# learningmatter-mit/surface-sampling

Measured on AMD Instinct MI355X. Metric: MC energy-evaluations/sec (SrTiO3(001) ~250-atom slabs, 3-model PaiNN ensemble E+F incl. neighbor list), higher is better.
Workload: dtype f32 via fp16x2-split MFMA (3 products), fp32 accumulate; neighbor decisions f64; 1 GPU; SrTiO3(001) PaiNN x3, 256 batched independent chains per GPU (BASELINE configs[3]), 248-272 atoms/chain; chains_per_gpu=256, atoms_per_gpu=66503, edges_per_gpu=2747786, slots_per_gpu=2836316, models=3, streams_per_gpu=2, parallelism=one GPU, no collective

## Files before the change

surface-sampling_amd/csrc/painn.hip:

```cpp
#include "vssr_internal.h"

namespace vssr {

constexpr int T = NODE_TILE;
constexpr int RB = 21;
constexpr int ECHUNK = 16;
constexpr float PI_F = 3.14159265358979323846f;

__device__ inline float sigmoidf_(float x) { return 1.f / (1.f + expf(-x)); }
__device__ inline float swishf_(float x) { return x * sigmoidf_(x); }
__device__ inline float dswishf_(float x) {
    float sg = sigmoidf_(x);
    return sg * fmaf(x, 1.f - sg, 1.f);
}

__global__ void __launch_bounds__(128) k_embed(int N, const int *__restrict__ Z, const ModelW *__restrict__ MW,
                                               float *__restrict__ s0, float *__restrict__ v0) {
    int i = blockIdx.x, m = blockIdx.y, f = threadIdx.x;
    const ModelW &W = MW[m];
    size_t a = (size_t)m * N + i;
    s0[a * F + f] = W.embed[(size_t)Z[i] * F + f];
    v0[(a * 3 + 0) * F + f] = 0.f;
    v0[(a * 3 + 1) * F + f] = 0.f;
    v0[(a * 3 + 2) * F + f] = 0.f;
// ... 509 lines not shown
    return painn_alloc_results(h);
}

int painn_alloc_results(vssr_handle *h) {
    const size_t N = h->n_atoms, M = h->n_models;
    if (h->d_energy.ensure(sizeof(float) * h->n_cfg) || h->d_energy_std.ensure(sizeof(float) * h->n_cfg) ||
        h->d_energy_models.ensure(sizeof(float) * h->n_cfg * M) || h->d_energy64.ensure(sizeof(double) * h->n_cfg * (2 + M)) ||
        h->d_forces.ensure(sizeof(float) * 3 * N) ||
        h->d_forces_std.ensure(sizeof(float) * 3 * N) || h->d_e_atoms.ensure(sizeof(float) * N))
        return set_err(h, VSSR_E_NOMEM, "result buffers: out of device memory");
    if (h->d_sat.bytes < sizeof(unsigned) * h->n_cfg || h->d_sat_out.bytes < sizeof(unsigned) * h->n_cfg) {
        if (h->d_sat.ensure(sizeof(unsigned) * h->n_cfg) || h->d_sat_out.ensure(sizeof(unsigned) * h->n_cfg))
            return set_err(h, VSSR_E_NOMEM, "saturation flags: out of device memory");
        VSSR_HIP(h, hipMemsetAsync(h->d_sat.p, 0, h->d_sat.bytes, h->stream));
        VSSR_HIP(h, hipMemsetAsync(h->d_sat_out.p, 0, h->d_sat_out.bytes, h->stream));
    }
    return VSSR_OK;
}

int painn_run(vssr_handle *h, uint32_t want) {
    if (h->painn_general) return painn_gen_run(h, want);
    const int N = h->n_atoms, M = h->n_models, L = h->num_conv, H = h->readout_hidden;
    hipStream_t st = h->stream;
    h->h_sat_valid = false;
    int rc = build_neighbors(h, (double)h->cutoff);
    if (rc) return rc;
    rc = painn_alloc_state(h);
    if (rc) return rc;
    StateView &sv = h->sv;
    sv.e_excl = h->d_excl.as<float>();
    const GraphView G = graph_view(h);
    const ActiveView &av = G.act;
    const ModelW *MW = h->model_table.as<ModelW>();
    const int *counters = h->d_counters.as<int>();
    const int *Z = h->d_Z.as<int>();
    dim3 blk(128);
    dim3 g_atom(N, M), g_tile((N + T - 1) / T, M);
    Profiler &P = h->prof;
    const bool l0_fact = h->l0_enabled && h->l0_nz > 0;
    const int n_groups = painn_gbar_groups(h);
    const bool partial = n_groups > 1;
    const int layer_sets = partial ? L - 1 : 1, per_set = n_groups / layer_sets;
    const int *cls_list[EDGE_MFMA_CLASSES];
    const int *bcls_list[EDGE_MFMA_BCLASSES];
    {
        int o = 0;
        for (int c = 0; c < EDGE_MFMA_CLASSES; o += h->n_class[c], ++c) cls_list[c] = h->d_class_list.as<int>() + o;
        for (int c = 0; c < EDGE_MFMA_BCLASSES; o += h->n_bclass[c], ++c) bcls_list[c] = h->d_class_list.as<int>() + o;
    }
    const int n_gather = h->n_class[EDGE_CLASS_GATHER];
    const bool keep = h->upd_save && (want & VSSR_WANT_FORCES) && readout_mfma_supported(H);
    auto save_of = [&](int l) -> void * { return keep ? (char *)h->d_upd_save.p + update_save_bytes(N, M) * (size_t)l : nullptr; };
    h->l0_used = l0_fact;

    if (!l0_fact) {
        P.begin(KC_EMBED, st);
        hipLaunchKernelGGL(k_embed, g_atom, blk, 0, st, N, Z, MW, sv.s_in[0], sv.v_in[0]);
        P.end(st);
    }
    for (int l = 0; l < L; ++l) {
        if (l == 0 && l0_fact) {
            P.begin(KC_L0_FWD, st);
            rc = l0_run_forward(h, G, sv.s_msg[0], sv.v_msg[0]);
            if (rc) return rc;
            P.end(st);
            P.begin(KC_UPDATE_FWD, st);
            launch_update_fwd_mfma(st, N, M, l, av, MW, sv.s_msg[l], sv.v_msg[l], sv.s_in[l + 1],
                                   (l + 1 < L || h->debug_keep) ? sv.v_in[l + 1] : nullptr, l + 1 < L ? sv.phi[l + 1] : nullptr, save_of(l));
            P.end(st);
            continue;
        }
        if (l == 0) {
            P.begin(KC_MSG_MLP, st);
            launch_msg_mlp_mfma(st, N, M, l, av, MW, sv.s_in[l], sv.phi[l]);
            P.end(st);
        }
        P.begin(KC_EDGE_FWD, st);
        if (l == 0)
            hipLaunchKernelGGL(k_edge_fwd<true>, g_atom, blk, 0, st, N, l, MW, G, counters, h->cutoff, h->excl_vol,
                               h->excl_sigma, h->excl_power, sv.s_in[l], sv.v_in[l], sv.phi[l], sv.s_msg[l],
                               sv.v_msg[l], -1);
        else {
            for (int cls = 0; cls < EDGE_MFMA_CLASSES; ++cls)
                launch_edge_fwd_mfma(st, cls, N, cls_list[cls], h->n_class[cls], M, l, h->max_class_atoms[cls], MW, G, counters,
                                     (int)(h->slot_cap - 1), sv.s_in[l], sv.v_in[l], sv.phi[l], sv.s_msg[l], sv.v_msg[l],
                                     (cls == EDGE_CLASS_FS4 && h->fwd_two_pass) ? h->d_bundle_sub.as<int4>() : (const int4 *)nullptr,
                                     h->fwd_two_pass, h->sub_chunk_fwd ? h->sub_chunk_fwd : sub_chunk_max(h->fwd_two_pass));
            if (n_gather)
                hipLaunchKernelGGL(k_edge_fwd<false>, g_atom, blk, 0, st, N, l, MW, G, counters, h->cutoff, h->excl_vol,
                                   h->excl_sigma, h->excl_power, sv.s_in[l], sv.v_in[l], sv.phi[l], sv.s_msg[l],
                                   sv.v_msg[l], (int)EDGE_BCLASS_GATHER);
        }
        P.end(st);
        P.begin(KC_UPDATE_FWD, st);
        launch_update_fwd_mfma(st, N, M, l, av, MW, sv.s_msg[l], sv.v_msg[l], sv.s_in[l + 1],
                               (l + 1 < L || h->debug_keep) ? sv.v_in[l + 1] : nullptr, l + 1 < L ? sv.phi[l + 1] : nullptr, save_of(l));
        P.end(st);
    }
    const bool fused = readout_mfma_supported(H);
    const bool want_forces = (want & VSSR_WANT_FORCES) != 0;
    const float *e_excl = h->excl_vol ? sv.e_excl : (const float *)nullptr;
    if (!(fused && want_forces)) {
        P.begin(KC_READOUT, st);
        if (fused) launch_readout_mfma(st, N, M, av, MW, sv.s_in[L], e_excl, sv.e_atom);
        else
            hipLaunchKernelGGL(k_readout, g_tile, blk, 0, st, N, H, av, MW, sv.s_in[L], sv.e_excl, h->excl_vol, sv.e_atom,
                               sv.sbar);
        P.end(st);
    }

    if (want_forces) {
        float *sb_buf[2] = {sv.sbar_msg, sv.sbar};
        for (int l = L - 1; l >= 0; --l) {
            float *sbar_msg_l = fused ? sb_buf[(L - 1 - l) & 1] : sv.sbar_msg;
            const float *sbar_msg_up = sb_buf[(L - l) & 1];
            P.begin(KC_UPDATE_BWD, st);
            if (!fused)
                launch_update_bwd_mfma(st, N, M, l, 0, (int)(l == L - 1), av, MW, sv.s_msg[l], sv.v_msg[l], sv.sbar, sv.vbar,
                                       nullptr, nullptr, nullptr, nullptr, sbar_msg_l, sv.vbar_msg, nullptr);
            else if (l == L - 1)
                launch_update_bwd_mfma(st, N, M, l, 1, 1, av, MW, sv.s_msg[l], sv.v_msg[l], nullptr, sv.vbar, sv.s_in[L], nullptr,
                                       e_excl, sv.e_atom, sbar_msg_l, sv.vbar_msg, save_of(l));
            else
                launch_update_bwd_mfma(st, N, M, l, 2, 0, av, MW, sv.s_msg[l], sv.v_msg[l], sbar_msg_up, sv.vbar, sv.s_in[l + 1],
                                       sv.phibar, nullptr, nullptr, sbar_msg_l, sv.vbar_msg, save_of(l));
            P.end(st);
            sv.sbar_msg_l0 = sbar_msg_l;
            P.begin((l == 0 && l0_fact) ? KC_L0_BWD : KC_EDGE_BWD, st);
            int accumulate = (l != L - 1);
            if (l == 0 && l0_fact) {
                rc = l0_run_reverse(h, G, (int)(L == 1), (int)partial, sbar_msg_l, sv.vbar_msg, sv.gbar);
                if (rc) return rc;
            } else if (l == 0)
                hipLaunchKernelGGL(k_edge_bwd<true>, g_atom, blk, 0, st, N, l, accumulate, MW, G, counters,
                                   h->cutoff, h->excl_vol, h->excl_sigma, h->excl_power, sv.v_in[l], sv.phi[l],
                                   sbar_msg_l, sv.vbar_msg, sv.phibar, sv.vbar, sv.gbar,
                                   (long long)h->slot_cap, -1, (int)partial);
            else {
                for (int cls = 0; cls < EDGE_MFMA_BCLASSES; ++cls)
                    launch_edge_bwd_mfma(st, cls, N, bcls_list[cls], h->n_bclass[cls], M, l, h->max_bclass_atoms[cls], MW, G, counters,
                                         (int)(h->slot_cap - 1), sv.v_in[l], sv.phi[l], sbar_msg_l, sv.vbar_msg, sv.phibar, sv.vbar,
                                         h->d_gpart.as<float>(), (long long)h->slot_cap, n_groups, (L - 1 - l) * per_set,
                                         cls == EDGE_BCLASS_FS16P ? h->d_bundle_subb.as<int4>() : (const int4 *)nullptr,
                                         h->sub_chunk_bwd ? h->sub_chunk_bwd : sub_chunk_max_bwd());
                if (n_gather)
                    hipLaunchKernelGGL(k_edge_bwd<false>, g_atom, blk, 0, st, N, l, accumulate, MW, G, counters,
                                       h->cutoff, h->excl_vol, h->excl_sigma, h->excl_power, sv.v_in[l], sv.phi[l],
                                       sbar_msg_l, sv.vbar_msg, sv.phibar, sv.vbar, sv.gbar,
                                       (long long)h->slot_cap, (int)EDGE_BCLASS_GATHER, 0);
            }
            P.end(st);
            if (l > 0 && !fused) {
                P.begin(KC_MSG_MLP_BWD, st);
                launch_msg_mlp_bwd_mfma(st, N, M, l, av, MW, sv.s_in[l], sv.phibar, sv.sbar_msg, sv.sbar);
                P.end(st);
            }
        }
    }
    P.begin(KC_FINALIZE, st);
    if (want_forces && partial) {
        const int uni = h->active_mask ? 0 : h->n_bclass[EDGE_BCLASS_FS16] + h->n_bclass[EDGE_BCLASS_FS16P] == h->n_cfg ? 8 : h->n_bclass[EDGE_BCLASS_FS8] == h->n_cfg ? 16
                        : h->n_bclass[EDGE_BCLASS_FS4] == h->n_cfg ? 32 : 0;
        const dim3 grid = uni ? dim3((unsigned)((h->slot_cap + 255) / 256), 1) : dim3(h->n_cfg, 12);
        hipLaunchKernelGGL(k_reduce_gpart, grid, dim3(256), 0, st, M, n_groups, layer_sets, G, counters, h->d_gpart.as<float>(),
                           sv.gbar, (long long)h->slot_cap, uni);
    }
    painn_finalize(h, G, want);
    P.end(st);
    VSSR_HIP(h, hipGetLastError());
    return VSSR_OK;
}

void painn_finalize(vssr_handle *h, const GraphView &G, uint32_t want) {
    const int N = h->n_atoms, M = h->n_models;
    hipStream_t st = h->stream;
    if (want & VSSR_WANT_FORCES)
        hipLaunchKernelGGL(k_finalize_forces, dim3((N + 3) / 4), dim3(256), 0, st, N, M, G, h->d_counters.as<int>(), h->sv.gbar,
                           (long long)h->slot_cap, h->units_per_ev, h->d_forces.as<float>(), h->d_forces_std.as<float>());
// ... 17 lines not shown
```

surface-sampling_amd/csrc/painn_node_mfma.hip:

```cpp
#include "mfma16.h"

#ifdef PHASE_TIMING
__device__ unsigned long long g_phase[64];
#define PH_INIT unsigned long long ph_t = wall_clock64();
#define PH_RESET ph_t = wall_clock64();
#define PH(k) { const unsigned long long ph_n = wall_clock64(); if (threadIdx.x == 0) atomicAdd(&g_phase[k], ph_n - ph_t); ph_t = wall_clock64(); }
extern "C" int vssr_debug_phases(unsigned long long *out, int reset) {
    if (hipMemcpyFromSymbol(out, HIP_SYMBOL(g_phase), sizeof(unsigned long long) * 64) != hipSuccess) return -1;
    if (reset) { unsigned long long z[64] = {}; if (hipMemcpyToSymbol(HIP_SYMBOL(g_phase), z, sizeof(z)) != hipSuccess) return -1; }
    return 0;
}
#else
#define PH_INIT
#define PH_RESET
#define PH(k)
#endif

namespace vssr {

template <int NRT, int NCT>
struct GemmShape {
    static constexpr int NT = NRT * NCT, NACC = NT >= 3 ? 1 : 2;
};
template <int NRT, int NCT, int NPRE>
// ... 228 lines not shown
    zero_acc(a1);
    const f32x4 b1v = gload4f(W.b1 + L.col0);
    __builtin_amdgcn_sched_barrier(0);
    {
        const uint4 *wp[1] = {WTILE(W1, L.w, F)};
        gemm16<F, 2, 1>(xs, wp, h1);
        const uint4 *wq[1] = {WTILE(W2t, L.w, F3)};
        gemm16<F3, 2, 1>(pb, wq, a1);
    }
    __syncthreads();
    {
        const f32x4 b = b1v;
#pragma unroll
        for (int t = 0; t < 2; ++t) {
            f32x4 hv;
#pragma unroll
            for (int i = 0; i < 4; ++i) hv[i] = a1[t][0][i] * dswish(h1[t][0][i] + b[i]);
            store_split4(xs, L.row(t), L.col0, hv, sat);
        }
    }
    __syncthreads();
    f32x4 acc[2][1];
    zero_acc(acc);
    const uint4 *wp[1] = {WTILE(W1t, L.w, F)};
    gemm16<F, 2, 1>(xs, wp, acc);
#pragma unroll
    for (int t = 0; t < 2; ++t) {
        const int a = a0 + L.row(t);
        if (a < N)
            *reinterpret_cast<f32x4 *>(sbar_in + (mN + a) * F + L.col0) = gload4f(sbar_msg + (mN + a) * F + L.col0) + acc[t][0];
    }
    sat.commit(av, a0, N);
}

template <int RT>
struct UpdLds {
    static constexpr int TA = 16 * RT;
    static constexpr int OFF_VT = 0;
    static constexpr int OFF_HS = plane_halves(3 * TA, F);
    static constexpr int OFF_AS = OFF_HS + plane_halves(TA, 2 * F);
    static constexpr int HALVES = OFF_AS + plane_halves(TA, F);
    static_assert(plane_halves(TA, F3) <= OFF_HS, "qb overlays vt");
    static_assert(plane_halves(3 * TA, 2 * F) <= HALVES, "[Ubar | Vbar] overlays the whole region");
};

template <int RT>
struct UpdRegs {
    f32x4 uv[3 * RT][2];
    f32x4 h3[RT];
    f32x4 gate[RT][2];
    f32x4 nrm[RT], inner[RT];
};

template <int RT, int PHB, int PF, class Sat>
__device__ __forceinline__ void update_forward(const LayerW &W, _Float16 *ldsh, const LaneGeo &L, UpdRegs<RT> &R, Sat &sat) {
    constexpr int TA = 16 * RT, OFF_VT = UpdLds<RT>::OFF_VT, OFF_HS = UpdLds<RT>::OFF_HS, OFF_AS = UpdLds<RT>::OFF_AS;
    const Planes vt = make_planes(ldsh + OFF_VT, 3 * TA, F), hs = make_planes(ldsh + OFF_HS, TA, 2 * F),
                 as_ = make_planes(ldsh + OFF_AS, TA, F);
    zero_acc(R.uv);
    PH_INIT
    {
        const uint4 *wp[2] = {WTILE(U, L.w, F), WTILE(V, L.w, F)};
        gemm16<F, 3 * RT, 2, PF>(vt, wp, R.uv);
    }
    PH(PHB + 1)
#pragma unroll
    for (int t = 0; t < RT; ++t) {
#pragma unroll
        for (int i = 0; i < 4; ++i) {
            float n2 = 0.f, in = 0.f;
#pragma unroll
            for (int x = 0; x < 3; ++x) {
                const float vv = R.uv[RT * x + t][1][i];
                n2 += fmaf(vv, vv, 1e-15f);
                in = fmaf(R.uv[RT * x + t][0][i], vv, in);
            }
            R.nrm[t][i] = sqrtf(n2);
            R.inner[t][i] = in;
        }
        store_split4(hs, L.row(t), F + L.col0, R.nrm[t], sat);
    }
    PH(PHB + 2)
    __syncthreads();
    PH(PHB + 3)
    {
        f32x4 acc[RT][1];
        zero_acc(acc);
        const uint4 *wp[1] = {WTILE(W3, L.w, 2 * F)};
        const f32x4 b = gload4f(W.b3 + L.col0);
        __builtin_amdgcn_sched_barrier(0);
        gemm16<2 * F, RT, 1, PF>(hs, wp, acc);
#pragma unroll
        for (int t = 0; t < RT; ++t) {
            R.h3[t] = acc[t][0] + b;
            f32x4 sw;
#pragma unroll
            for (int i = 0; i < 4; ++i) sw[i] = swish(R.h3[t][i]);
            store_split4(as_, L.row(t), L.col0, sw, sat);
        }
    }
    PH(PHB + 4)
    __syncthreads();
    PH(PHB + 5)
    {
        zero_acc(R.gate);
        const uint4 *wp[2] = {WTILE(W4, L.w, F), WTILE(W4, NW + L.w, F)};
        f32x4 b4[2];
#pragma unroll
        for (int c = 0; c < 2; ++c) b4[c] = gload4f(W.b4 + c * F + L.col0);
        __builtin_amdgcn_sched_barrier(0);
        gemm16<F, RT, 2, PF>(as_, wp, R.gate);
#pragma unroll
        for (int c = 0; c < 2; ++c) {
            const f32x4 b = b4[c];
#pragma unroll
            for (int t = 0; t < RT; ++t) R.gate[t][c] += b;
        }
    }
    PH(PHB + 6)
}

template <int RT, class Sat>
__device__ __forceinline__ void load_update_v(_Float16 *ldsh, const float *__restrict__ v_msg, size_t mN, int a0, int N, Sat &sat) {
    constexpr int TA = 16 * RT;
    const Planes vt = make_planes(ldsh + UpdLds<RT>::OFF_VT, 3 * TA, F);
    load_rows_split<3 * TA>(vt, 0, [&](int row) {
        int x = row / TA, a = min(a0 + (row % TA), N - 1);
        return v_msg + ((mN + a) * 3 + x) * F;
    }, sat);
}
template <int RT, class Sat>
__device__ __forceinline__ void load_update_s(_Float16 *ldsh, const float *__restrict__ s_msg, size_t mN, int a0, int N, Sat &sat) {
    constexpr int TA = 16 * RT;
    const Planes hs = make_planes(ldsh + UpdLds<RT>::OFF_HS, TA, 2 * F);
    load_rows_split<TA>(hs, 0, [&](int row) { return s_msg + (mN + min(a0 + row, N - 1)) * F; }, sat);
}

constexpr int CF_XS = plane_halves(3 * TA, F);
constexpr int CF_LDS_HALVES = CF_XS + plane_halves(TA, F);
static_assert(2 * plane_halves(TA, F) <= CF_XS, "|Vv| and swish planes overlay the v tile");
static_assert(4 * TA * FT * sizeof(float) <= CF_LDS_HALVES * sizeof(_Float16), "output tile overlays the planes");
#ifndef UPD_SAVE_LATE
#define UPD_SAVE_LATE 1
#endif
constexpr int UPD_SAVE_UV = 0, UPD_SAVE_H3 = 12, UPD_SAVE_GATE = 14, UPD_SAVE_REGS = 18;
__device__ __forceinline__ f32x4 &save_slot(f32x4 *save, int m, int k) {
    return save[(((size_t)m * gridDim.x + blockIdx.x) * UPD_SAVE_REGS + k) * NTHREADS + threadIdx.x];
}
size_t update_save_bytes(int N, int M) { return sizeof(f32x4) * (size_t)M * ((N + TA - 1) / TA) * UPD_SAVE_REGS * NTHREADS; }

template <int TAIL>
__global__ void __launch_bounds__(NTHREADS) __attribute__((amdgpu_waves_per_eu(2, 2)))
k_update_fwd_mfma(int N, int l, ActiveView av, const ModelW *__restrict__ MW, const float *__restrict__ s_msg,
                  const float *__restrict__ v_msg, float *__restrict__ s_out, float *__restrict__ v_out,
                  float *__restrict__ phi_next, f32x4 *__restrict__ save) {
    extern __shared__ __attribute__((aligned(16))) _Float16 ldsh[];
    constexpr bool NOV = TAIL == 2;
// ... 234 lines not shown
                es = fmaf(w6[i], swish(hval[i]), es);
                hb[i] = w6[i] * dswish(hval[i]);
            }
            if (WANT_SBAR) store_split4(hp, L.row(t), L.col0, hb, sat);
            es = xrow_sum_f32(es);
            if (lane < 16) red[L.w * TA + L.row(t)] = es;
        }
    }
    __syncthreads();
    if (threadIdx.x < TA) {
        const int atom = a0 + threadIdx.x;
        if (atom < N) {
            float e = gload1f(W.b6);
#pragma unroll
            for (int k = 0; k < NCW; ++k) e += red[k * TA + threadIdx.x];
            if (e_excl) e += e_excl[atom];
            e_atom[mN + atom] = e;
        }
    }
    if (WANT_SBAR) {
        f32x4 acc[RT][1];
        zero_acc(acc);
        const uint4 *wp[1] = {W.qW5t + (size_t)L.w * 4 * RH};
        gemm16<RH, RT, 1>(hp, wp, acc);
#pragma unroll
        for (int t = 0; t < RT; ++t) sb[t] = acc[t][0];
    }
}

__global__ void __launch_bounds__(NTHREADS)
k_readout_mfma(int N, ActiveView av, const ModelW *__restrict__ MW, const float *__restrict__ s, const float *__restrict__ e_excl,
               float *__restrict__ e_atom) {
    extern __shared__ __attribute__((aligned(16))) _Float16 ldsh[];
    const int m = blockIdx.y, a0 = blockIdx.x * TA;
    if (!av.tile(min(a0, N - 1), min(a0 + TA - 1, N - 1))) return;
    const LaneGeo L;
    SatTrack sat;
    const size_t mN = (size_t)m * N;
    const Planes xs = make_planes(ldsh, TA, F), hp = make_planes(ldsh + plane_halves(TA, F), TA, RH);
    float *red = reinterpret_cast<float *>(ldsh + plane_halves(TA, F) + plane_halves(TA, RH));
    load_rows_split<TA>(xs, 0, [&](int row) { return s + (mN + min(a0 + row, N - 1)) * F; }, sat);
    __syncthreads();
    f32x4 sb[2];
    readout_head<2, false>(MW[m], xs, hp, red, L, a0, N, mN, e_excl, e_atom, sb, sat);
    sat.commit(av, a0, N);
}

template <int MODE, int RT, bool SAVED = false>
__global__ void __launch_bounds__(NTHREADS) __attribute__((amdgpu_waves_per_eu(RT == 1 ? 4 : 2, RT == 1 ? 4 : 2)))
k_update_bwd_mfma(int N, int l, int vbar_is_zero, ActiveView av, const ModelW *__restrict__ MW, const float *__restrict__ s_msg,
                  const float *__restrict__ v_msg, const float *__restrict__ sbar_src, const float *__restrict__ vbar,
                  const float *__restrict__ s_next, const float *__restrict__ phibar, const float *__restrict__ e_excl,
                  float *__restrict__ e_atom, float *__restrict__ sbar_msg, float *__restrict__ vbar_msg,
                  const f32x4 *__restrict__ save) {
    static_assert(!SAVED || RT == 2, "the saved layout is that of the 32-atom forward kernel");
    extern __shared__ __attribute__((aligned(16))) _Float16 ldsh[];
    constexpr int TA = 16 * RT, OFF_VT = UpdLds<RT>::OFF_VT, OFF_AS = UpdLds<RT>::OFF_AS, UPD_LDS_HALVES = UpdLds<RT>::HALVES;
    const int m = blockIdx.y, a0 = blockIdx.x * TA;
    if (!av.tile(min(a0, N - 1), min(a0 + TA - 1, N - 1))) return;
    const LaneGeo L;
    constexpr int BPF = MODE == 0 ? 0 : UPD_PF;
    SatNone unwatched;
    const LayerW &W = MW[m].layer[l];
    const size_t mN = (size_t)m * N;
    PH_INIT
    f32x4 sb[RT];
    if (MODE != 1) {
#pragma unroll
        for (int t = 0; t < RT; ++t) sb[t] = gload4f(sbar_src + (mN + min(a0 + L.row(t), N - 1)) * F + L.col0);
    }
    float *VB = reinterpret_cast<float *>(ldsh + UPD_LDS_HALVES);
    if (MODE == 1) vbar_is_zero = 1;
    if (!vbar_is_zero) {
        constexpr int NIT = 3 * TA * (F / 4) / NTHREADS;
        float4 vv[NIT];
#pragma unroll
        for (int it = 0; it < NIT; ++it) {
            const int idx = threadIdx.x + it * NTHREADS, row = idx >> 5, c4 = idx & 31;
            vv[it] = *reinterpret_cast<const float4 *>(vbar + ((mN + min(a0 + row % TA, N - 1)) * 3 + row / TA) * F + 4 * c4);
        }
#pragma unroll
        for (int it = 0; it < NIT; ++it) {
            const int idx = threadIdx.x + it * NTHREADS, row = idx >> 5, c4 = idx & 31;
            *reinterpret_cast<float4 *>(VB + row * FT + 4 * c4) = vv[it];
        }
    }
    UpdRegs<RT> R;
    auto load_saved = [&]() {
        const f32x4 *sv = save + (((size_t)m * gridDim.x + blockIdx.x) * UPD_SAVE_REGS) * NTHREADS + threadIdx.x;
#pragma unroll
        for (int j = 0; j < 3 * RT; ++j)
#pragma unroll
            for (int c = 0; c < 2; ++c) R.uv[j][c] = gload4f(reinterpret_cast<const float *>(sv + (size_t)(UPD_SAVE_UV + 2 * j + c) * NTHREADS));
#pragma unroll
        for (int t = 0; t < RT; ++t) {
            R.h3[t] = gload4f(reinterpret_cast<const float *>(sv + (size_t)(UPD_SAVE_H3 + t) * NTHREADS));
#pragma unroll
            for (int c = 0; c < 2; ++c) R.gate[t][c] = gload4f(reinterpret_cast<const float *>(sv + (size_t)(UPD_SAVE_GATE + 2 * t + c) * NTHREADS));
        }
    };
    if (!SAVED) load_update_s<RT>(ldsh, s_msg, mN, a0, N, unwatched);
    else load_saved();
    if (MODE == 0) {
        load_update_v<RT>(ldsh, v_msg, mN, a0, N, unwatched);
        __syncthreads();
    } else if (MODE == 1) {
        if (!SAVED) load_update_v<RT>(ldsh, v_msg, mN, a0, N, unwatched);
        const Planes xs = make_planes(ldsh + OFF_AS, TA, F);
        const Planes hp = make_planes(ldsh + UPD_LDS_HALVES, TA, RH);
        float *red = reinterpret_cast<float *>(ldsh + UPD_LDS_HALVES + plane_halves(TA, RH));
        {
            SatTrack satc;
            load_rows_split<TA>(xs, 0, [&](int row) { return s_next + (mN + min(a0 + row, N - 1)) * F; }, satc);
            satc.commit(av, a0, N);
        }
        __syncthreads();
        PH(40)
        {
            SatTrack sate;
            readout_head<RT, true>(MW[m], xs, hp, red, L, a0, N, mN, e_excl, e_atom, sb, sate);
            sate.commit(av, a0, N);
        }
        PH(41)
    } else {
        const LayerW &Wn = MW[m].layer[l + 1];
        const Planes xs = make_planes(ldsh + OFF_AS, TA, F), pb = make_planes(ldsh + OFF_VT, TA, F3);
        load_rows_split<TA>(xs, 0, [&](int row) { return s_next + (mN + min(a0 + row, N - 1)) * F; }, unwatched);
        {
            SatTrack satc;
#pragma unroll
            for (int c = 0; c < 3; ++c)
                load_rows_split<TA>(pb, c * F, [&](int row) { return phibar + (mN + min(a0 + row, N - 1)) * F3 + c * F; }, satc);
            satc.commit(av, a0, N);
        }
        __syncthreads();
        PH(42)
        f32x4 h1[RT][1], a1[RT][1];
        zero_acc(h1);
        zero_acc(a1);
        const f32x4 b1n = gload4f(Wn.b1 + L.col0);
        __builtin_amdgcn_sched_barrier(0);
        {
            const uint4 *wp[1] = {Wn.qW1 + (size_t)L.w * 4 * F};
            gemm16<F, RT, 1, BPF>(xs, wp, h1);
            const uint4 *wq[1] = {Wn.qW2t + (size_t)L.w * 4 * F3};
            gemm16<F3, RT, 1, BPF>(pb, wq, a1);
        }
        PH(43)
        __syncthreads();
        if (!SAVED) load_update_v<RT>(ldsh, v_msg, mN, a0, N, unwatched);
        PH(44)
        {
            const f32x4 b = b1n;
            SatTrack sate;
#pragma unroll
            for (int t = 0; t < RT; ++t) {
                f32x4 hv;
#pragma unroll
                for (int i = 0; i < 4; ++i) hv[i] = a1[t][0][i] * dswish(h1[t][0][i] + b[i]);
                store_split4(xs, L.row(t), L.col0, hv, sate);
            }
            sate.commit(av, a0, N);
        }
        __syncthreads();
        f32x4 acc[RT][1];
        zero_acc(acc);
        const uint4 *wp[1] = {Wn.qW1t + (size_t)L.w * 4 * F};
        gemm16<F, RT, 1, BPF>(xs, wp, acc);
#pragma unroll
        for (int t = 0; t < RT; ++t) sb[t] += acc[t][0];
        PH(45)
    }
    PH(16)
    if constexpr (!SAVED) {
        update_forward<RT, 16, BPF>(W, ldsh, L, R, unwatched);
    } else {
#pragma unroll
        for (int t = 0; t < RT; ++t)
#pragma unroll
            for (int i = 0; i < 4; ++i) {
                float in = 0.f;
#pragma unroll
                for (int x = 0; x < 3; ++x) in = fmaf(R.uv[RT * x + t][0][i], R.uv[RT * x + t][1][i], in);
                R.inner[t][i] = in;
            }
        __syncthreads();
    }
    PH_RESET
    const Planes qb = make_planes(ldsh + OFF_VT, TA, F3);
    SatTrack sat;
#pragma unroll
    for (int t = 0; t < RT; ++t) {
        const int row = L.row(t);
        f32x4 abar_vv = {0.f, 0.f, 0.f, 0.f};
        if (!vbar_is_zero) {
#pragma unroll
            for (int x = 0; x < 3; ++x) {
                const f32x4 vb = *reinterpret_cast<const f32x4 *>(VB + (x * TA + row) * FT + L.col0);
#pragma unroll
                for (int i = 0; i < 4; ++i) abar_vv[i] = fmaf(vb[i], R.uv[RT * x + t][0][i], abar_vv[i]);
            }
        }
        store_split4(qb, row, L.col0, abar_vv, sat);
        store_split4(qb, row, F + L.col0, sb[t] * R.inner[t], sat);
        store_split4(qb, row, 2 * F + L.col0, sb[t], sat);
    }
    sat.commit(av, a0, N);
    sat = SatTrack();
    PH(23)
    __syncthreads();
    PH(24)
    const Planes hb = make_planes(ldsh + OFF_AS, TA, F);
    {
        f32x4 acc[RT][1];
        zero_acc(acc);
        const uint4 *wp[1] = {WTILE(W4t, L.w, F3)};
        gemm16<F3, RT, 1, BPF>(qb, wp, acc);
#pragma unroll
        for (int t = 0; t < RT; ++t) {
            f32x4 hv;
#pragma unroll
            for (int i = 0; i < 4; ++i) hv[i] = acc[t][0][i] * dswish(R.h3[t][i]);
            store_split4(hb, L.row(t), L.col0, hv, sat);
        }
        sat.commit(av, a0, N);
        sat = SatTrack();
    }
    PH(25)
// ... 79 lines not shown
void pack_mfma_tiles16(const float *Wsrc, int rows, int K, unsigned *dst) {
    auto split2 = [](float x, unsigned (&p)[2]) {
        const _Float16 h = (_Float16)x;
        const _Float16 l = (_Float16)(x - (float)h);
        unsigned short hb, lb;
        memcpy(&hb, &h, 2);
        memcpy(&lb, &l, 2);
        p[0] = hb; p[1] = lb;
    };
    const int ntile = rows / 16, nq = K / 32;
    for (int tile = 0; tile < ntile; ++tile)
        for (int q = 0; q < nq; ++q)
            for (int lane = 0; lane < 64; ++lane)
                for (int j = 0; j < 4; ++j) {
                    const size_t row = (size_t)tile * 16 + (lane & 15);
                    const int k = 32 * q + 8 * (lane >> 4) + 2 * j;
                    unsigned p0[2], p1[2];
                    split2(Wsrc[row * K + k], p0);
                    split2(Wsrc[row * K + k + 1], p1);
                    for (int pc = 0; pc < 2; ++pc)
                        dst[((((size_t)tile * nq + q) * 2 + pc) * 64 + lane) * 4 + j] = p0[pc] | (p1[pc] << 16);
                }
}

size_t node_mfma_lds_bytes(int which) {
    switch (which) {
        case 0: return sizeof(_Float16) * 2 * plane_halves(TA, F);
        case 1: return sizeof(_Float16) * (plane_halves(TA, F) + plane_halves(TA, F3));
        case 4: return sizeof(_Float16) * (plane_halves(TA, F) + plane_halves(TA, RH)) + sizeof(float) * (RH / 16) * TA;
        case 6: return 96 * 1024;
        default: return sizeof(_Float16) * UpdLds<2>::HALVES + sizeof(float) * 3 * TA * FT;
    }
}
static_assert(sizeof(_Float16) * plane_halves(16, RH) + sizeof(float) * (RH / 16) * 16 <= sizeof(float) * 3 * 16 * FT,
              "readout scratch fits the vbar region");

static_assert(sizeof(_Float16) * (CF_LDS_HALVES + plane_halves(TA, F)) <= 96 * 1024, "update fwd LDS request");

bool readout_mfma_supported(int hidden) { return hidden == RH; }

int node_mfma_init(vssr_handle *h) {
    VSSR_HIP(h, hipFuncSetAttribute((const void *)k_msg_mlp_mfma<2, 0>, hipFuncAttributeMaxDynamicSharedMemorySize, 96 * 1024));
    VSSR_HIP(h, hipFuncSetAttribute((const void *)k_msg_mlp_bwd_mfma, hipFuncAttributeMaxDynamicSharedMemorySize,
                                    (int)node_mfma_lds_bytes(1)));
    VSSR_HIP(h, hipFuncSetAttribute((const void *)k_update_fwd_mfma<0>, hipFuncAttributeMaxDynamicSharedMemorySize,
                                    (int)node_mfma_lds_bytes(6)));
    VSSR_HIP(h, hipFuncSetAttribute((const void *)k_update_fwd_mfma<1>, hipFuncAttributeMaxDynamicSharedMemorySize,
                                    (int)node_mfma_lds_bytes(6)));
    VSSR_HIP(h, hipFuncSetAttribute((const void *)k_update_fwd_mfma<2>, hipFuncAttributeMaxDynamicSharedMemorySize,
                                    (int)node_mfma_lds_bytes(6)));
#define SET_UPD(MODE)                                                                                                     \
    VSSR_HIP(h, hipFuncSetAttribute((const void *)k_update_bwd_mfma<MODE, 2>, hipFuncAttributeMaxDynamicSharedMemorySize, \
                                    (int)node_mfma_lds_bytes(3)));
    SET_UPD(0) SET_UPD(1) SET_UPD(2)
#undef SET_UPD
    VSSR_HIP(h, hipFuncSetAttribute((const void *)k_update_bwd_mfma<1, 2, true>, hipFuncAttributeMaxDynamicSharedMemorySize,
                                    (int)node_mfma_lds_bytes(3)));
    VSSR_HIP(h, hipFuncSetAttribute((const void *)k_update_bwd_mfma<2, 2, true>, hipFuncAttributeMaxDynamicSharedMemorySize,
                                    (int)node_mfma_lds_bytes(3)));
    VSSR_HIP(h, hipFuncSetAttribute((const void *)k_readout_mfma, hipFuncAttributeMaxDynamicSharedMemorySize,
                                    (int)node_mfma_lds_bytes(4)));
    return VSSR_OK;
}

void launch_msg_mlp_mfma(hipStream_t st, int N, int M, int l, const ActiveView &av, const ModelW *MW, const float *s_in,
                         float *phi) {
    hipLaunchKernelGGL((k_msg_mlp_mfma<2, 0>), dim3((N + TA - 1) / TA, M), dim3(NTHREADS), node_mfma_lds_bytes(0), st, N, l, av, MW,
                       s_in, phi);
}
void launch_msg_mlp_bwd_mfma(hipStream_t st, int N, int M, int l, const ActiveView &av, const ModelW *MW, const float *s_in,
                             const float *phibar, const float *sbar_msg, float *sbar_in) {
    hipLaunchKernelGGL(k_msg_mlp_bwd_mfma, dim3((N + TA - 1) / TA, M), dim3(NTHREADS), node_mfma_lds_bytes(1), st, N, l, av, MW,
                       s_in, phibar, sbar_msg, sbar_in);
}
void launch_update_fwd_mfma(hipStream_t st, int N, int M, int l, const ActiveView &av, const ModelW *MW, const float *s_msg,
                            const float *v_msg, float *s_out, float *v_out, float *phi_next, void *save) {
    f32x4 *sv = reinterpret_cast<f32x4 *>(save);
    if (phi_next)
        hipLaunchKernelGGL(k_update_fwd_mfma<1>, dim3((N + TA - 1) / TA, M), dim3(NTHREADS), node_mfma_lds_bytes(6), st, N, l,
                           av, MW, s_msg, v_msg, s_out, v_out, phi_next, sv);
    else if (!v_out && !sv)
        hipLaunchKernelGGL(k_update_fwd_mfma<2>, dim3((N + TA - 1) / TA, M), dim3(NTHREADS), node_mfma_lds_bytes(6), st, N, l,
                           av, MW, s_msg, v_msg, s_out, v_out, phi_next, sv);
    else
        hipLaunchKernelGGL(k_update_fwd_mfma<0>, dim3((N + TA - 1) / TA, M), dim3(NTHREADS), node_mfma_lds_bytes(6), st, N, l,
                           av, MW, s_msg, v_msg, s_out, v_out, phi_next, sv);
}
void launch_readout_mfma(hipStream_t st, int N, int M, const ActiveView &av, const ModelW *MW, const float *s,
                         const float *e_excl, float *e_atom) {
    hipLaunchKernelGGL(k_readout_mfma, dim3((N + TA - 1) / TA, M), dim3(NTHREADS), node_mfma_lds_bytes(4), st, N, av, MW, s,
                       e_excl, e_atom);
}
void launch_update_bwd_mfma(hipStream_t st, int N, int M, int l, int mode, int vbar_is_zero, const ActiveView &av, const ModelW *MW,
                            const float *s_msg, const float *v_msg, const float *sbar_src, const float *vbar,
                            const float *s_next, const float *phibar, const float *e_excl, float *e_atom,
                            float *sbar_msg, float *vbar_msg, const void *save) {
    const f32x4 *sv = reinterpret_cast<const f32x4 *>(save);
    if (mode == 1) vbar_is_zero = 1;
#if defined(UPD_BWD_RT) && UPD_BWD_RT == 1
    if (!sv && mode != 0) {
        const dim3 grid1((N + 15) / 16, M), blk1(NTHREADS);
        const size_t lds1 = sizeof(_Float16) * UpdLds<1>::HALVES + sizeof(float) * 3 * 16 * FT;
        static bool once = [] {
            (void)hipFuncSetAttribute((const void *)k_update_bwd_mfma<1, 1, false>, hipFuncAttributeMaxDynamicSharedMemorySize, 80 * 1024);
            (void)hipFuncSetAttribute((const void *)k_update_bwd_mfma<2, 1, false>, hipFuncAttributeMaxDynamicSharedMemorySize, 80 * 1024);
            return true;
        }();
        (void)once;
        if (mode == 1)
            hipLaunchKernelGGL((k_update_bwd_mfma<1, 1, false>), grid1, blk1, lds1, st, N, l, vbar_is_zero, av, MW, s_msg, v_msg, sbar_src,
                               vbar, s_next, phibar, e_excl, e_atom, sbar_msg, vbar_msg, sv);
        else
            hipLaunchKernelGGL((k_update_bwd_mfma<2, 1, false>), grid1, blk1, lds1, st, N, l, vbar_is_zero, av, MW, s_msg, v_msg, sbar_src,
                               vbar, s_next, phibar, e_excl, e_atom, sbar_msg, vbar_msg, sv);
        return;
    }
#endif
    const dim3 grid((N + TA - 1) / TA, M), blk(NTHREADS);
    const size_t lds = node_mfma_lds_bytes(3);
#define LAUNCH_UPD(MODE, SAVED)                                                                                             \
    hipLaunchKernelGGL((k_update_bwd_mfma<MODE, 2, SAVED>), grid, blk, lds, st, N, l, vbar_is_zero, av, MW, s_msg, v_msg, sbar_src, \
                       vbar, s_next, phibar, e_excl, e_atom, sbar_msg, vbar_msg, sv)
    if (mode == 1) { if (sv) LAUNCH_UPD(1, true); else LAUNCH_UPD(1, false); }
    else if (mode == 2) { if (sv) LAUNCH_UPD(2, true); else LAUNCH_UPD(2, false); }
    else LAUNCH_UPD(0, false);
#undef LAUNCH_UPD
}

}
```

surface-sampling_amd/csrc/vssr_internal.h:

```cpp
#pragma once

#include <hip/hip_runtime.h>

#include <cstdint>
#include <cstdio>
#include <cstdlib>
#include <cstring>
#include <memory>
#include <string>
#include <utility>
#include <vector>

#include "../../include/vssr_eval.h"

namespace vssr {

constexpr int F = 128;
constexpr int F3 = 3 * F;
constexpr int MAX_LAYERS = 4;
constexpr int MAX_MODELS = 8;
constexpr int RB_MAX = 24;
constexpr int NODE_TILE = 8;
constexpr int L0_MAX_SPECIES = 8;

// ... 417 lines not shown
int gmm_fit_append_host(vssr_handle *h, int64_t n_rows, const double *x);
int gmm_fit_append_f32(vssr_handle *h, hipStream_t st, int64_t n_rows, const float *emb_dev);
int gmm_fit_append_f64p(vssr_handle *h, hipStream_t st, int64_t n_rows, const double *x_dev);
int gmm_fit_set_init(vssr_handle *h, const double *means, const double *weights, const double *precisions, const int32_t *labels);
int gmm_fit_run(vssr_handle *h, vssr_gmm_fit_result *res);
int gmm_fit_params(vssr_handle *h, double *weights, double *means, double *covariances, double *prec_chol);
int gmm_fit_copy_scorer(vssr_handle *h, vssr_handle *g);
int gmm_fit_centered_cov(vssr_handle *h, hipStream_t st, const double *X, int n, int D, int Dp, const double *mean, const double *denom,
                         DevBuf &part, double *cov);
int cluster_pca(vssr_handle *h, vssr_cluster_pca_result *res);
int cluster_pca_params(vssr_handle *h, double *mean, double *components, double *explained_variance, double *ratio);
int cluster_projected(vssr_handle *h, int64_t first, int64_t n_rows, double *xr);
int cluster_set_points(vssr_handle *h, int64_t n, const double *pts);
int cluster_linkage(vssr_handle *h, double *Z, int32_t *n_rounds);
int cluster_pad_dims(int d);
int tersoff_stress(vssr_handle *h);
int eam_stress(vssr_handle *h);
int sw_stress(vssr_handle *h);
struct PotView;
void ewald_run(vssr_handle *h, const PotView &V);
int ewald_stress(vssr_handle *h);
int pair_stress(vssr_handle *h);
struct Evaluator {
    bool f64;
    int (*run)(vssr_handle *h, uint32_t want);
    int (*stress)(vssr_handle *h);
    double (*cutoff)(const vssr_handle *h);
};
const Evaluator &evaluator(const vssr_handle *h);
inline bool is_analytic(const vssr_handle *h) { return evaluator(h).f64; }
void eam_build_spline(const double *f, int n, double delta, double *spl );
int relax_fire(vssr_handle *h, const vssr_fire_params &p, const uint8_t *fixed_host, uint32_t want);
int relax_bfgs(vssr_handle *h, const vssr_bfgs_params &p, const uint8_t *fixed_host, uint32_t want);
int relax_begin(vssr_handle *h, const uint8_t *fixed_host, int steps_ints_per_chain, const uint8_t *&fixed);
int relax_regrow(vssr_handle *h, int cap, long long &it, int window);
int relax_cg(vssr_handle *h, const vssr_cg_params *cp, const uint8_t *fixed_host, uint32_t want);
int relax_bfgsls(vssr_handle *h, const vssr_bfgsls_params *bp, const uint8_t *fixed_host, uint32_t want);
bool chain_min_supported(const vssr_handle *h);
int chain_min_cg(vssr_handle *h, const vssr_cg_params *cp, const uint8_t *fixed_host, uint32_t want);
int node_mfma_init(vssr_handle *h);
void launch_msg_mlp_mfma(hipStream_t st, int N, int M, int l, const ActiveView &av, const ModelW *MW, const float *s_in,
                         float *phi);
void launch_msg_mlp_bwd_mfma(hipStream_t st, int N, int M, int l, const ActiveView &av, const ModelW *MW, const float *s_in,
                             const float *phibar, const float *sbar_msg, float *sbar_in);
void launch_update_fwd_mfma(hipStream_t st, int N, int M, int l, const ActiveView &av, const ModelW *MW, const float *s_msg,
                            const float *v_msg, float *s_out, float *v_out, float *phi_next, void *save);
size_t update_save_bytes(int N, int M);
bool readout_mfma_supported(int hidden);
void launch_readout_mfma(hipStream_t st, int N, int M, const ActiveView &av, const ModelW *MW, const float *s, const float *e_excl,
                         float *e_atom);
void launch_update_bwd_mfma(hipStream_t st, int N, int M, int l, int mode, int vbar_is_zero, const ActiveView &av, const ModelW *MW,
                            const float *s_msg, const float *v_msg, const float *sbar_src, const float *vbar,
                            const float *s_next, const float *phibar, const float *e_excl, float *e_atom,
                            float *sbar_msg, float *vbar_msg, const void *save);
void pack_mfma_tiles16(const float *Wsrc, int rows, int K, unsigned *dst );
void build_wd16(const float *Wd, const float *bd, unsigned *dst );
void l0_build_tables(const float *blob_embed, const float *W1, const float *b1, const float *W2, const float *b2,
                     const float *Wd, const float *bd, int n_embed, float *A, float *At);
void l0_pack_tables(const float *A, int n_embed, unsigned *A16, unsigned *At16);
size_t l0_packed_dwords(int n_embed);
int l0_mfma_init(vssr_handle *h);
int l0_run_forward(vssr_handle *h, const GraphView &G, float *s_msg, float *v_msg);
int l0_run_reverse(vssr_handle *h, const GraphView &G, int first_write, int fresh_mfma, const float *sbar_msg, const float *vbar_msg,
                   float4 *gbar);
int edge_mfma_init(vssr_handle *h);
enum { EDGE_CLASS_FS16 = 0, EDGE_CLASS_FS16M = 1, EDGE_CLASS_FS8 = 2, EDGE_CLASS_FS4 = 3, EDGE_CLASS_GATHER = 4, EDGE_CLASSES = 5,
       EDGE_MFMA_CLASSES = 4 };
enum { EDGE_BCLASS_FS16 = 0, EDGE_BCLASS_FS8 = 1, EDGE_BCLASS_FS4 = 2, EDGE_BCLASS_FS16P = 3, EDGE_BCLASS_GATHER = 4, EDGE_BCLASSES = 5,
       EDGE_MFMA_BCLASSES = 4 };
__host__ __device__ constexpr int edge_bclass_slices(int c) { return (c == EDGE_BCLASS_FS16 || c == EDGE_BCLASS_FS16P) ? 8 : c == EDGE_BCLASS_FS8 ? 16 : c == EDGE_BCLASS_FS4 ? 32 : 1; }
int edge_bclass_of(int n_atoms);
int edge_class_of(int n_atoms);
constexpr int SUB_MAX_PASSES = 4;
__host__ __device__ constexpr int sub_chunk_max(int width) { return width == 16 ? 400 : 784; }
__host__ __device__ constexpr int sub_chunk_max_bwd() { return 550; }
__host__ __device__ constexpr int sub_passes(int n_atoms, int chunk_max) { return (n_atoms + chunk_max - 1) / chunk_max; }
__host__ __device__ constexpr int sub_chunk(int n_atoms, int chunk_max) { return (n_atoms + sub_passes(n_atoms, chunk_max) - 1) / sub_passes(n_atoms, chunk_max); }
int edge_class_groups(int cls);
void launch_edge_bwd_mfma(hipStream_t st, int cls, int N, const int *list, int n_list, int M, int l, int max_atoms,
                          const ModelW *MW, const GraphView &G, const int *counters, int zero_slot,
                          const float *v_in, const float *phi, const float *sbar_msg, const float *vbar_msg,
                          float *phibar, float *vbar_in, float *gpart, long long slot_cap, int n_groups, int group_off,
                          const int4 *bundle_sub, int sub_chunk);
void launch_edge_fwd_mfma(hipStream_t st, int cls, int N, const int *list, int n_list, int M, int l, int max_atoms, const ModelW *MW,
                          const GraphView &G, const int *counters, int zero_slot, const float *s_in, const float *v_in,
                          const float *phi, float *s_msg, float *v_msg, const int4 *bundle_sub, int sub_width, int sub_chunk);

}
```

Before: 24440 evaluations/s.

## Fuse last-layer forward update and readout into the first backward update kernel

When forces are requested and update intermediates are not saved, the final layer's forward update kernel is skipped. A new mode-3 backward kernel recomputes that update in-tile, including the scalar residual and gate output, writes s_last, runs the readout head and then continues into the backward pass. This saves one kernel launch plus the global round trip of the last layer's s/v outputs and readout inputs. In exchange the fused kernel carries more LDS scratch and register pressure, and it only applies when the keep/save path is off.

```diff
diff --git a/surface-sampling_amd/csrc/painn.hip b/surface-sampling_amd/csrc/painn.hip
--- a/surface-sampling_amd/csrc/painn.hip
+++ b/surface-sampling_amd/csrc/painn.hip
@@ -585,6 +585,15 @@
     const bool keep = h->upd_save && (want & VSSR_WANT_FORCES) && readout_mfma_supported(H);
     auto save_of = [&](int l) -> void * { return keep ? (char *)h->d_upd_save.p + update_save_bytes(N, M) * (size_t)l : nullptr; };
     h->l0_used = l0_fact;
+    const bool fuse_last = readout_mfma_supported(H) && (want & VSSR_WANT_FORCES) && !keep;
+    auto update_fwd = [&](int l) {
+        const bool last = l + 1 == L;
+        if (last && fuse_last && !h->debug_keep) return;
+        P.begin(KC_UPDATE_FWD, st);
+        launch_update_fwd_mfma(st, N, M, l, av, MW, sv.s_msg[l], sv.v_msg[l], sv.s_in[l + 1],
+                               (!last || h->debug_keep) ? sv.v_in[l + 1] : nullptr, !last ? sv.phi[l + 1] : nullptr, save_of(l));
+        P.end(st);
+    };
 
     if (!l0_fact) {
         P.begin(KC_EMBED, st);
@@ -597,10 +606,7 @@
             rc = l0_run_forward(h, G, sv.s_msg[0], sv.v_msg[0]);
             if (rc) return rc;
             P.end(st);
-            P.begin(KC_UPDATE_FWD, st);
-            launch_update_fwd_mfma(st, N, M, l, av, MW, sv.s_msg[l], sv.v_msg[l], sv.s_in[l + 1],
-                                   (l + 1 < L || h->debug_keep) ? sv.v_in[l + 1] : nullptr, l + 1 < L ? sv.phi[l + 1] : nullptr, save_of(l));
-            P.end(st);
+            update_fwd(l);
             continue;
         }
         if (l == 0) {
@@ -625,10 +631,7 @@
                                    sv.v_msg[l], (int)EDGE_BCLASS_GATHER);
         }
         P.end(st);
-        P.begin(KC_UPDATE_FWD, st);
-        launch_update_fwd_mfma(st, N, M, l, av, MW, sv.s_msg[l], sv.v_msg[l], sv.s_in[l + 1],
-                               (l + 1 < L || h->debug_keep) ? sv.v_in[l + 1] : nullptr, l + 1 < L ? sv.phi[l + 1] : nullptr, save_of(l));
-        P.end(st);
+        update_fwd(l);
     }
     const bool fused = readout_mfma_supported(H);
     const bool want_forces = (want & VSSR_WANT_FORCES) != 0;
@@ -650,13 +653,16 @@
             P.begin(KC_UPDATE_BWD, st);
             if (!fused)
                 launch_update_bwd_mfma(st, N, M, l, 0, (int)(l == L - 1), av, MW, sv.s_msg[l], sv.v_msg[l], sv.sbar, sv.vbar,
-                                       nullptr, nullptr, nullptr, nullptr, sbar_msg_l, sv.vbar_msg, nullptr);
+                                       nullptr, nullptr, nullptr, nullptr, sbar_msg_l, sv.vbar_msg, nullptr, nullptr);
+            else if (l == L - 1 && fuse_last)
+                launch_update_bwd_mfma(st, N, M, l, 3, 1, av, MW, sv.s_msg[l], sv.v_msg[l], nullptr, sv.vbar, nullptr, nullptr,
+                                       e_excl, sv.e_atom, sbar_msg_l, sv.vbar_msg, sv.s_in[L], nullptr);
             else if (l == L - 1)
                 launch_update_bwd_mfma(st, N, M, l, 1, 1, av, MW, sv.s_msg[l], sv.v_msg[l], nullptr, sv.vbar, sv.s_in[L], nullptr,
-                                       e_excl, sv.e_atom, sbar_msg_l, sv.vbar_msg, save_of(l));
+                                       e_excl, sv.e_atom, sbar_msg_l, sv.vbar_msg, nullptr, save_of(l));
             else
                 launch_update_bwd_mfma(st, N, M, l, 2, 0, av, MW, sv.s_msg[l], sv.v_msg[l], sbar_msg_up, sv.vbar, sv.s_in[l + 1],
-                                       sv.phibar, nullptr, nullptr, sbar_msg_l, sv.vbar_msg, save_of(l));
+                                       sv.phibar, nullptr, nullptr, sbar_msg_l, sv.vbar_msg, nullptr, save_of(l));
             P.end(st);
             sv.sbar_msg_l0 = sbar_msg_l;
             P.begin((l == 0 && l0_fact) ? KC_L0_BWD : KC_EDGE_BWD, st);
diff --git a/surface-sampling_amd/csrc/painn_node_mfma.hip b/surface-sampling_amd/csrc/painn_node_mfma.hip
--- a/surface-sampling_amd/csrc/painn_node_mfma.hip
+++ b/surface-sampling_amd/csrc/painn_node_mfma.hip
@@ -304,8 +304,20 @@
     f32x4 nrm[RT], inner[RT];
 };
 
-template <int RT, int PHB, int PF, class Sat>
-__device__ __forceinline__ void update_forward(const LayerW &W, _Float16 *ldsh, const LaneGeo &L, UpdRegs<RT> &R, Sat &sat) {
+struct SatUnwatched {
+    __device__ __forceinline__ SatNone begin() const { return SatNone(); }
+    __device__ __forceinline__ void end(const SatNone &) const {}
+};
+struct SatWatched {
+    const ActiveView &av;
+    int a0, N;
+    __device__ __forceinline__ SatTrack begin() const { return SatTrack(); }
+    __device__ __forceinline__ void end(const SatTrack &t) const { t.commit(av, a0, N); }
+};
+
+template <int RT, int PHB, int PF, bool FULL, class Scope>
+__device__ __forceinline__ void update_forward(const LayerW &W, _Float16 *ldsh, const LaneGeo &L, UpdRegs<RT> &R, f32x4 (&ass)[RT],
+                                               const Scope &scope) {
     constexpr int TA = 16 * RT, OFF_VT = UpdLds<RT>::OFF_VT, OFF_HS = UpdLds<RT>::OFF_HS, OFF_AS = UpdLds<RT>::OFF_AS;
     const Planes vt = make_planes(ldsh + OFF_VT, 3 * TA, F), hs = make_planes(ldsh + OFF_HS, TA, 2 * F),
                  as_ = make_planes(ldsh + OFF_AS, TA, F);
@@ -316,21 +328,25 @@
         gemm16<F, 3 * RT, 2, PF>(vt, wp, R.uv);
     }
     PH(PHB + 1)
-#pragma unroll
-    for (int t = 0; t < RT; ++t) {
-#pragma unroll
-        for (int i = 0; i < 4; ++i) {
-            float n2 = 0.f, in = 0.f;
-#pragma unroll
-            for (int x = 0; x < 3; ++x) {
-                const float vv = R.uv[RT * x + t][1][i];
-                n2 += fmaf(vv, vv, 1e-15f);
-                in = fmaf(R.uv[RT * x + t][0][i], vv, in);
-            }
-            R.nrm[t][i] = sqrtf(n2);
-            R.inner[t][i] = in;
-        }
-        store_split4(hs, L.row(t), F + L.col0, R.nrm[t], sat);
+    {
+        auto sat = scope.begin();
+#pragma unroll
+        for (int t = 0; t < RT; ++t) {
+#pragma unroll
+            for (int i = 0; i < 4; ++i) {
+                float n2 = 0.f, in = 0.f;
+#pragma unroll
+                for (int x = 0; x < 3; ++x) {
+                    const float vv = R.uv[RT * x + t][1][i];
+                    n2 += fmaf(vv, vv, 1e-15f);
+                    in = fmaf(R.uv[RT * x + t][0][i], vv, in);
+                }
+                R.nrm[t][i] = sqrtf(n2);
+                R.inner[t][i] = in;
+            }
+            store_split4(hs, L.row(t), F + L.col0, R.nrm[t], sat);
+        }
+        scope.end(sat);
     }
     PH(PHB + 2)
     __syncthreads();
@@ -341,7 +357,15 @@
         const uint4 *wp[1] = {WTILE(W3, L.w, 2 * F)};
         const f32x4 b = gload4f(W.b3 + L.col0);
         __builtin_amdgcn_sched_barrier(0);
-        gemm16<2 * F, RT, 1, PF>(hs, wp, acc);
+        if constexpr (FULL) {
+            const Planes hn = Planes{hs.h + F, hs.l + F, hs.ld};
+            const uint4 *wn[1] = {WTILE(W3, L.w, 2 * F) + (F / 32) * 2 * 64};
+            gemm16<F, RT, 1, PF>(hs, wp, acc);
+            gemm16<F, RT, 1, PF>(hn, wn, acc);
+        } else {
+            gemm16<2 * F, RT, 1, PF>(hs, wp, acc);
+        }
+        auto sat = scope.begin();
 #pragma unroll
         for (int t = 0; t < RT; ++t) {
             R.h3[t] = acc[t][0] + b;
@@ -350,11 +374,27 @@
             for (int i = 0; i < 4; ++i) sw[i] = swish(R.h3[t][i]);
             store_split4(as_, L.row(t), L.col0, sw, sat);
         }
+        scope.end(sat);
     }
     PH(PHB + 4)
     __syncthreads();
     PH(PHB + 5)
-    {
+    if constexpr (FULL) {
+        f32x4 g3[RT][3];
+        zero_acc(g3);
+        const uint4 *wp[3] = {WTILE(W4, L.w, F), WTILE(W4, NW + L.w, F), WTILE(W4, 2 * NW + L.w, F)};
+        f32x4 b4[3];
+#pragma unroll
+        for (int c = 0; c < 3; ++c) b4[c] = gload4f(W.b4 + c * F + L.col0);
+        __builtin_amdgcn_sched_barrier(0);
+        gemm16<F, RT, 3, PF>(as_, wp, g3);
+#pragma unroll
+        for (int t = 0; t < RT; ++t) {
+            R.gate[t][0] = g3[t][0] + b4[0];
+            R.gate[t][1] = g3[t][1] + b4[1];
+            ass[t] = g3[t][2] + b4[2];
+        }
+    } else {
         zero_acc(R.gate);
         const uint4 *wp[2] = {WTILE(W4, L.w, F), WTILE(W4, NW + L.w, F)};
         f32x4 b4[2];
@@ -695,8 +735,11 @@
                   const float *__restrict__ v_msg, const float *__restrict__ sbar_src, const float *__restrict__ vbar,
                   const float *__restrict__ s_next, const float *__restrict__ phibar, const float *__restrict__ e_excl,
                   float *__restrict__ e_atom, float *__restrict__ sbar_msg, float *__restrict__ vbar_msg,
-                  const f32x4 *__restrict__ save) {
+                  float *__restrict__ s_last, const f32x4 *__restrict__ save) {
     static_assert(!SAVED || RT == 2, "the saved layout is that of the 32-atom forward kernel");
+    constexpr bool FUSED = MODE == 3;
+    static_assert(!FUSED || (!SAVED && RT == 2), "the fused last block runs its own forward pass on 32-atom tiles");
+    static_assert(MODE != 1 || SAVED, "without stored intermediates the last layer is MODE 3");
     extern __shared__ __attribute__((aligned(16))) _Float16 ldsh[];
     constexpr int TA = 16 * RT, OFF_VT = UpdLds<RT>::OFF_VT, OFF_AS = UpdLds<RT>::OFF_AS, UPD_LDS_HALVES = UpdLds<RT>::HALVES;
     const int m = blockIdx.y, a0 = blockIdx.x * TA;
@@ -708,12 +751,16 @@
     const size_t mN = (size_t)m * N;
     PH_INIT
     f32x4 sb[RT];
-    if (MODE != 1) {
+    if (MODE != 1 && !FUSED) {
 #pragma unroll
         for (int t = 0; t < RT; ++t) sb[t] = gload4f(sbar_src + (mN + min(a0 + L.row(t), N - 1)) * F + L.col0);
     }
     float *VB = reinterpret_cast<float *>(ldsh + UPD_LDS_HALVES);
-    if (MODE == 1) vbar_is_zero = 1;
+    if (MODE == 1 || FUSED) vbar_is_zero = 1;
+    float *SR = VB + (plane_halves(TA, RH) / 2 + (RH / 16) * TA);
+    static_assert(!FUSED || ((plane_halves(TA, RH) / 2 + (RH / 16) * TA) % 4 == 0 &&
+                             plane_halves(TA, RH) / 2 + (RH / 16) * TA + TA * FT <= 3 * TA * FT),
+                  "readout scratch + fp32 residual tile fit the vbar region");
     if (!vbar_is_zero) {
         constexpr int NIT = 3 * TA * (F / 4) / NTHREADS;
         float4 vv[NIT];
@@ -742,30 +789,43 @@
             for (int c = 0; c < 2; ++c) R.gate[t][c] = gload4f(reinterpret_cast<const float *>(sv + (size_t)(UPD_SAVE_GATE + 2 * t + c) * NTHREADS));
         }
     };
-    if (!SAVED) load_update_s<RT>(ldsh, s_msg, mN, a0, N, unwatched);
+    auto readout = [&](const Planes &xs) {
+        const Planes hp = make_planes(ldsh + UPD_LDS_HALVES, TA, RH);
+        float *red = reinterpret_cast<float *>(ldsh + UPD_LDS_HALVES + plane_halves(TA, RH));
+        PH(40)
+        SatTrack sate;
+        readout_head<RT, true>(MW[m], xs, hp, red, L, a0, N, mN, e_excl, e_atom, sb, sate);
+        sate.commit(av, a0, N);
+        PH(41)
+    };
+    if (FUSED) {
+        float4 keep_s[TA * (F / 4) / NTHREADS];
+        SatTrack satc;
+        rows_request<TA>([&](int row) { return s_msg + (mN + min(a0 + row, N - 1)) * F; }, keep_s);
+        load_update_v<RT>(ldsh, v_msg, mN, a0, N, satc);
+        rows_store_split<TA>(make_planes(ldsh + UpdLds<RT>::OFF_HS, TA, 2 * F), 0, keep_s, satc);
+        satc.commit(av, a0, N);
+#pragma unroll
+        for (int it = 0; it < TA * (F / 4) / NTHREADS; ++it) {
+            const int idx = threadIdx.x + it * NTHREADS;
+            *reinterpret_cast<float4 *>(SR + (idx >> 5) * FT + 4 * (idx & 31)) = keep_s[it];
+        }
+        __syncthreads();
+    } else if (!SAVED) load_update_s<RT>(ldsh, s_msg, mN, a0, N, unwatched);
     else load_saved();
     if (MODE == 0) {
         load_update_v<RT>(ldsh, v_msg, mN, a0, N, unwatched);
         __syncthreads();
     } else if (MODE == 1) {
-        if (!SAVED) load_update_v<RT>(ldsh, v_msg, mN, a0, N, unwatched);
         const Planes xs = make_planes(ldsh + OFF_AS, TA, F);
-        const Planes hp = make_planes(ldsh + UPD_LDS_HALVES, TA, RH);
-        float *red = reinterpret_cast<float *>(ldsh + UPD_LDS_HALVES + plane_halves(TA, RH));
         {
             SatTrack satc;
             load_rows_split<TA>(xs, 0, [&](int row) { return s_next + (mN + min(a0 + row, N - 1)) * F; }, satc);
             satc.commit(av, a0, N);
         }
         __syncthreads();
-        PH(40)
-        {
-            SatTrack sate;
-            readout_head<RT, true>(MW[m], xs, hp, red, L, a0, N, mN, e_excl, e_atom, sb, sate);
-            sate.commit(av, a0, N);
-        }
-        PH(41)
-    } else {
+        readout(xs);
+    } else if (MODE == 2) {
         const LayerW &Wn = MW[m].layer[l + 1];
         const Planes xs = make_planes(ldsh + OFF_AS, TA, F), pb = make_planes(ldsh + OFF_VT, TA, F3);
         load_rows_split<TA>(xs, 0, [&](int row) { return s_next + (mN + min(a0 + row, N - 1)) * F; }, unwatched);
@@ -815,8 +875,27 @@
         PH(45)
     }
     PH(16)
-    if constexpr (!SAVED) {
-        update_forward<RT, 16, BPF>(W, ldsh, L, R, unwatched);
+    f32x4 ass[RT];
+    if constexpr (FUSED) {
+        update_forward<RT, 16, BPF, true>(W, ldsh, L, R, ass, SatWatched{av, a0, N});
+        const Planes xs = make_planes(ldsh + OFF_VT, TA, F);
+        {
+            SatTrack sato;
+#pragma unroll
+            for (int t = 0; t < RT; ++t) {
+                const int row = L.row(t), a = a0 + row;
+                f32x4 o = *reinterpret_cast<const f32x4 *>(SR + row * FT + L.col0);
+#pragma unroll
+                for (int i = 0; i < 4; ++i) o[i] += fmaf(R.gate[t][1][i], R.inner[t][i], ass[t][i]);
+                store_split4(xs, row, L.col0, o, sato);
+                if (a < N) *reinterpret_cast<f32x4 *>(s_last + (mN + a) * F + L.col0) = o;
+            }
+            sato.commit(av, a0, N);
+        }
+        __syncthreads();
+        readout(xs);
+    } else if constexpr (!SAVED) {
+        update_forward<RT, 16, BPF, false>(W, ldsh, L, R, ass, SatUnwatched{});
     } else {
 #pragma unroll
         for (int t = 0; t < RT; ++t)
@@ -1002,7 +1081,7 @@
 #define SET_UPD(MODE)                                                                                                     \
     VSSR_HIP(h, hipFuncSetAttribute((const void *)k_update_bwd_mfma<MODE, 2>, hipFuncAttributeMaxDynamicSharedMemorySize, \
                                     (int)node_mfma_lds_bytes(3)));
-    SET_UPD(0) SET_UPD(1) SET_UPD(2)
+    SET_UPD(0) SET_UPD(2) SET_UPD(3)
 #undef SET_UPD
     VSSR_HIP(h, hipFuncSetAttribute((const void *)k_update_bwd_mfma<1, 2, true>, hipFuncAttributeMaxDynamicSharedMemorySize,
                                     (int)node_mfma_lds_bytes(3)));
@@ -1044,25 +1123,20 @@
 void launch_update_bwd_mfma(hipStream_t st, int N, int M, int l, int mode, int vbar_is_zero, const ActiveView &av, const ModelW *MW,
                             const float *s_msg, const float *v_msg, const float *sbar_src, const float *vbar,
                             const float *s_next, const float *phibar, const float *e_excl, float *e_atom,
-                            float *sbar_msg, float *vbar_msg, const void *save) {
+                            float *sbar_msg, float *vbar_msg, float *s_last, const void *save) {
     const f32x4 *sv = reinterpret_cast<const f32x4 *>(save);
-    if (mode == 1) vbar_is_zero = 1;
+    if (mode == 1 || mode == 3) vbar_is_zero = 1;
 #if defined(UPD_BWD_RT) && UPD_BWD_RT == 1
-    if (!sv && mode != 0) {
+    if (!sv && mode == 2) {
         const dim3 grid1((N + 15) / 16, M), blk1(NTHREADS);
         const size_t lds1 = sizeof(_Float16) * UpdLds<1>::HALVES + sizeof(float) * 3 * 16 * FT;
         static bool once = [] {
-            (void)hipFuncSetAttribute((const void *)k_update_bwd_mfma<1, 1, false>, hipFuncAttributeMaxDynamicSharedMemorySize, 80 * 1024);
             (void)hipFuncSetAttribute((const void *)k_update_bwd_mfma<2, 1, false>, hipFuncAttributeMaxDynamicSharedMemorySize, 80 * 1024);
             return true;
         }();
         (void)once;
-        if (mode == 1)
-            hipLaunchKernelGGL((k_update_bwd_mfma<1, 1, false>), grid1, blk1, lds1, st, N, l, vbar_is_zero, av, MW, s_msg, v_msg, sbar_src,
-                               vbar, s_next, phibar, e_excl, e_atom, sbar_msg, vbar_msg, sv);
-        else
-            hipLaunchKernelGGL((k_update_bwd_mfma<2, 1, false>), grid1, blk1, lds1, st, N, l, vbar_is_zero, av, MW, s_msg, v_msg, sbar_src,
-                               vbar, s_next, phibar, e_excl, e_atom, sbar_msg, vbar_msg, sv);
+        hipLaunchKernelGGL((k_update_bwd_mfma<2, 1, false>), grid1, blk1, lds1, st, N, l, vbar_is_zero, av, MW, s_msg, v_msg, sbar_src,
+                           vbar, s_next, phibar, e_excl, e_atom, sbar_msg, vbar_msg, s_last, sv);
         return;
     }
 #endif
@@ -1070,9 +1144,10 @@
     const size_t lds = node_mfma_lds_bytes(3);
 #define LAUNCH_UPD(MODE, SAVED)                                                                                             \
     hipLaunchKernelGGL((k_update_bwd_mfma<MODE, 2, SAVED>), grid, blk, lds, st, N, l, vbar_is_zero, av, MW, s_msg, v_msg, sbar_src, \
-                       vbar, s_next, phibar, e_excl, e_atom, sbar_msg, vbar_msg, sv)
-    if (mode == 1) { if (sv) LAUNCH_UPD(1, true); else LAUNCH_UPD(1, false); }
+                       vbar, s_next, phibar, e_excl, e_atom, sbar_msg, vbar_msg, s_last, sv)
+    if (mode == 1) LAUNCH_UPD(1, true);
     else if (mode == 2) { if (sv) LAUNCH_UPD(2, true); else LAUNCH_UPD(2, false); }
+    else if (mode == 3) LAUNCH_UPD(3, false);
     else LAUNCH_UPD(0, false);
 #undef LAUNCH_UPD
 }
diff --git a/surface-sampling_amd/csrc/vssr_internal.h b/surface-sampling_amd/csrc/vssr_internal.h
--- a/surface-sampling_amd/csrc/vssr_internal.h
+++ b/surface-sampling_amd/csrc/vssr_internal.h
@@ -493,7 +493,7 @@
 void launch_update_bwd_mfma(hipStream_t st, int N, int M, int l, int mode, int vbar_is_zero, const ActiveView &av, const ModelW *MW,
                             const float *s_msg, const float *v_msg, const float *sbar_src, const float *vbar,
                             const float *s_next, const float *phibar, const float *e_excl, float *e_atom,
-                            float *sbar_msg, float *vbar_msg, const void *save);
+                            float *sbar_msg, float *vbar_msg, float *s_last, const void *save);
 void pack_mfma_tiles16(const float *Wsrc, int rows, int K, unsigned *dst );
 void build_wd16(const float *Wd, const float *bd, unsigned *dst );
 void l0_build_tables(const float *blob_embed, const float *W1, const float *b1, const float *W2, const float *b2,
```

Measured after the change: 24870 evaluations/s (median of 6 runs). 1.02x the previous value.
